# skokec/DAU-ConvNet

Measured on AMD Instinct MI355X. Metric: DAU fwd+bwd GSamples/s (N*H*W/s), higher is better.
Workload: dtype f32

## Files before the change

dau-convnet_amd/csrc/k_split_dot.hip:

```cpp
#include <algorithm>
#include <cfloat>

#include "dau_tiled.hpp"

namespace dau {

typedef _Float16 h8 __attribute__((ext_vector_type(8)));
typedef float f4s __attribute__((ext_vector_type(4)));

namespace {

constexpr int kSdWaves = 8;
constexpr int kSdAS = 2;
constexpr int kSdGT = 4;
constexpr int kSdSB = kSdWaves * kSdAS;
constexpr int kSdFB = 16;
constexpr int kSdR = 4;
constexpr int kSdRH = 4;
constexpr int kSdFlushItems = 16;
constexpr unsigned kVmcnt0 = 0x0F70, kVmcnt8 = 0x0F78;

inline size_t rup(size_t v, size_t a = 256) { return (v + a - 1) / a * a; }

struct SdGeom {
    int Hq, Wq, rq, cq, XTr, XTc, EYs, EXs, octs, nfb, nsb, ngb, items, chunks, per, NP;
};

SdGeom sd_geom(const SplitDotConfig& c) {
    const Shape& s = c.sh;
    SdGeom g{};
    g.Hq = (s.H + 1 + kSdRH - 1) / kSdRH * kSdRH;
    g.Wq = (s.W + 1 + c.RW - 1) / c.RW * c.RW;
    g.rq = g.Hq / kSdRH; g.cq = g.Wq / c.RW;
    g.XTr = g.Hq + 1; g.XTc = g.Wq + 1;
    g.EYs = g.Hq + 2 * kSdR; g.EXs = g.Wq + 2 * kSdR;
    g.octs = (s.N + 7) / 8;
    g.NP = (s.N + 1) / 2;
    g.nfb = (s.F + kSdFB - 1) / kSdFB;
    g.nsb = (s.S + kSdSB - 1) / kSdSB;
    g.ngb = (s.G + kSdGT - 1) / kSdGT;
    g.items = g.octs * g.rq * g.cq;
    const int per_chunk = g.nfb * g.nsb * g.ngb;
    int chunks = (1024 + per_chunk - 1) / per_chunk;
    chunks = std::max(1, std::min(chunks, g.items));
    g.per = (g.items + chunks - 1) / chunks;
    g.chunks = (g.items + g.per - 1) / g.per;
    return g;
}

struct SdLayout { size_t maxes_off, xk_off, xs_off, es_off, partial_off, total; };

SdLayout sd_layout(const SplitDotConfig& c, const SdGeom& g) {
    const Shape& s = c.sh;
    SdLayout l{};
    size_t off = 0;
    l.maxes_off = off; off += rup((size_t)(s.S * kNumK + s.F) * 4);
    l.xk_off = off; off += rup((size_t)g.NP * s.S * s.H * s.W * 32);
    l.xs_off = off; off += rup((size_t)g.octs * s.S * kNumK * g.XTr * g.XTc * 32 + 32);
    l.es_off = off; off += rup((size_t)g.octs * g.nfb * g.EYs * g.EXs * 256 * c.e_limbs);
    l.partial_off = off; off += rup((size_t)g.chunks * kNumK * s.S * s.G * s.F * 4);
    l.total = off;
    return l;
}

__device__ __forceinline__ int sd_shift(unsigned maxbits) {
    if (maxbits == 0u) return 0;
    const int e = (int)(maxbits >> 23) - 127;
    const int sh = 13 - e;
    return sh > 120 ? 120 : sh;
}

__device__ __forceinline__ bool finite_abs(float v, float* a) {
    *a = fabsf(v);
    return *a <= FLT_MAX;
}

#ifdef DAU_SD_STAGE_REF
__global__ void __launch_bounds__(256) sd_absmax_x_kernel(const float* __restrict__ xk, int NP, int S, int HW, int split,
                                                          unsigned* __restrict__ xmax, const Guard guard) {
    if (!guard_pass(guard)) return;
    const int s = blockIdx.x % S, part = blockIdx.x / S;
    float m[4] = {0.0f, 0.0f, 0.0f, 0.0f};
    const long per_np = (long)HW * 2;
    const long total = (long)NP * per_np;
    for (long i = part * 256L + threadIdx.x; i < total; i += 256L * split) {
        const long np = i / per_np, r = i - np * per_np;
        const float4 v = reinterpret_cast<const float4*>(xk + ((size_t)np * S + s) * HW * 8)[r];
        const int k0 = (int)(r & 1) * 2;
        float a;
        if (finite_abs(v.x, &a)) m[k0] = fmaxf(m[k0], a);
        if (finite_abs(v.y, &a)) m[k0] = fmaxf(m[k0], a);
        if (finite_abs(v.z, &a)) m[k0 + 1] = fmaxf(m[k0 + 1], a);
        if (finite_abs(v.w, &a)) m[k0 + 1] = fmaxf(m[k0 + 1], a);
    }
    __shared__ float red[4][256];
    for (int k = 0; k < 4; ++k) red[k][threadIdx.x] = m[k];
    __syncthreads();
    for (int w = 128; w >= 1; w >>= 1) {
        if ((int)threadIdx.x < w)
            for (int k = 0; k < 4; ++k) red[k][threadIdx.x] = fmaxf(red[k][threadIdx.x], red[k][threadIdx.x + w]);
        __syncthreads();
    }
    if (threadIdx.x < 4) atomicMax(&xmax[s * kNumK + threadIdx.x], __float_as_uint(red[threadIdx.x][0]));
}
#endif

__global__ void __launch_bounds__(256) sd_absmax_e_kernel(const float* __restrict__ dy, int N, int F, int HW, int split, int act,
                                                          unsigned* __restrict__ emax, const Guard guard) {
    if (!guard_pass(guard)) return;
    const int f = blockIdx.x % F, part = blockIdx.x / F;
    float m = 0.0f;
    const long total = (long)N * HW;
    for (long i = part * 256L + threadIdx.x; i < total; i += 256L * split) {
        const long n = i / HW, p = i - n * HW;
        float a;
        if (finite_abs(load_act(dy, ((long)n * F + f) * HW + p, act), &a)) m = fmaxf(m, a);
    }
    for (int o = 32; o >= 1; o >>= 1) m = fmaxf(m, __shfl_xor(m, o));
    if ((threadIdx.x & 63) == 0) atomicMax(&emax[f], __float_as_uint(m));
}

__global__ void __launch_bounds__(256) sd_absmax_nhwc_e_kernel(const float* __restrict__ dy, int N, int F, int HW, int split, int act,
                                                               unsigned* __restrict__ emax, const Guard guard) {
    if (!guard_pass(guard)) return;
    const int nfb = (F + 63) / 64;
    const int f = (blockIdx.x % nfb) * 64 + (threadIdx.x & 63), part = blockIdx.x / nfb;
    if (f >= F) return;
    float m = 0.0f;
    const long total = (long)N * HW;
    for (long i = part * 4L + (threadIdx.x >> 6); i < total; i += 4L * split) {
        float a;
        if (finite_abs(load_act(dy, i * F + f, act), &a)) m = fmaxf(m, a);
    }
    atomicMax(&emax[f], __float_as_uint(m));
}

__device__ __forceinline__ void split_limbs(float v, _Float16* hi, _Float16* lo) {
    const _Float16 h = (_Float16)v;
    const float hf = (float)h;
    *hi = h;
    *lo = (hf - hf == 0.0f) ? (_Float16)(v - hf) : (_Float16)0.0f;
}

__global__ void __launch_bounds__(256) sd_stage_x_kernel(const float* __restrict__ xk, const unsigned* __restrict__ xmax, int N,
                                                         int NP, int S, int H, int W, int octs, int XTr, int XTc,
                                                         h8* __restrict__ xs, const Guard guard) {
    if (!guard_pass(guard)) return;
    const long total = (long)octs * S * XTr * XTc;
    for (long idx = blockIdx.x * 256L + threadIdx.x; idx < total; idx += (long)gridDim.x * 256) {
        long t = idx;
        const int tx = (int)(t % XTc); t /= XTc;
        const int ty = (int)(t % XTr); t /= XTr;
        const int s = (int)(t % S);
        const int oct = (int)(t / S);
        const int y = ty - 1, x = tx - 1;
        const bool in = y >= 0 && y < H && x >= 0 && x < W;
        float v[4][8];
#pragma unroll
        for (int p = 0; p < 4; ++p) {
            const int np = oct * 4 + p;
            float4 a = make_float4(0.f, 0.f, 0.f, 0.f), b = a;
            if (in && np < NP) {
                const float4* src = reinterpret_cast<const float4*>(xk + ((((size_t)np * S + s) * H + y) * W + x) * 8);
                a = src[0]; b = src[1];
            }
            v[0][2 * p] = a.x; v[0][2 * p + 1] = a.y; v[1][2 * p] = a.z; v[1][2 * p + 1] = a.w;
            v[2][2 * p] = b.x; v[2][2 * p + 1] = b.y; v[3][2 * p] = b.z; v[3][2 * p + 1] = b.w;
        }
#pragma unroll
        for (int k = 0; k < 4; ++k) {
            const float sc = ldexpf(1.0f, sd_shift(xmax[s * kNumK + k]));
            h8 hi, lo;
#pragma unroll
            for (int i = 0; i < 8; ++i) {
                _Float16 h, l;
                split_limbs(v[k][i] * sc, &h, &l);
                hi[i] = h; lo[i] = l;
            }
            h8* dst = xs + ((((size_t)oct * S + s) * kNumK + k) * XTr * XTc + (size_t)ty * XTc + tx) * 2;
            dst[0] = hi; dst[1] = lo;
        }
    }
}

#ifndef DAU_SD_STAGE_REF
constexpr int kSeTX = 80;
__global__ void __launch_bounds__(256) sd_stage_e_kernel(const float* __restrict__ dy, const unsigned* __restrict__ emax, int N,
                                                         int F, int H, int W, int nfb, int EYs, int EXs, int nct, int TX,
                                                         int drop_col, int drop_row, int act, h8* __restrict__ es,
                                                         const Guard guard) {
    __shared__ h8 tile[kSeTX * 32];
    if (!guard_pass(guard)) return;
    int t = blockIdx.x;
    const int ct = t % nct; t /= nct;
    const int vy = t % EYs; t /= EYs;
    const int fb = t % nfb;
    const int oct = t / nfb;
    const int wlim = drop_col ? W - 1 : W, hlim = drop_row ? H - 1 : H;
    const int vx0 = ct * TX, nvx = min(TX, EXs - vx0);
    const int y = vy - (kSdR + 1);
    const int c0 = max(vx0, kSdR + 1), c1 = (y >= 0 && y < hlim) ? min(vx0 + nvx, kSdR + 1 + wlim) : c0;
    const int nd = max(c1 - c0, 0);
    for (int i = threadIdx.x; i < kSdFB * nd; i += 256) {
        const int fl = i / nd, vx = c0 + (i - fl * nd), x = vx - (kSdR + 1), lx = vx - vx0;
        const int f = fb * kSdFB + fl;
        const float sc = f < F ? ldexpf(1.0f, sd_shift(emax[f])) : 0.0f;
        float v[8];
#pragma unroll
        for (int n = 0; n < 8; ++n) {
            const int img = oct * 8 + n;
            v[n] = (f < F && img < N) ? load_act(dy, (((long)img * F + f) * H + y) * W + x, act) : 0.0f;
        }
        h8 hi, lo;
#pragma unroll
        for (int n = 0; n < 8; ++n) {
            _Float16 h, l;
            split_limbs(v[n] * sc, &h, &l);
            hi[n] = h; lo[n] = l;
        }
        tile[lx * 32 + (fl ^ (lx & 7))] = hi;
        tile[lx * 32 + ((kSdFB + fl) ^ (lx & 7))] = lo;
    }
    if (nd > 0) __syncthreads();
    h8* dst = es + ((((size_t)oct * nfb + fb) * EYs + vy) * EXs + vx0) * 32;
    for (int q = threadIdx.x; q < nvx * 32; q += 256) {
        const int lx = q >> 5, vx = vx0 + lx;
        h8 piece = {0, 0, 0, 0, 0, 0, 0, 0};
        if (vx >= c0 && vx < c1) piece = tile[lx * 32 + ((q & 31) ^ (lx & 7))];
        dst[q] = piece;
    }
}
#else
__global__ void __launch_bounds__(256) sd_stage_e_kernel(const float* __restrict__ dy, const unsigned* __restrict__ emax, int N,
                                                         int F, int H, int W, int octs, int nfb, int EYs, int EXs, int drop_col,
                                                         int drop_row, int act, int nhwc, h8* __restrict__ es, const Guard guard) {
    if (!guard_pass(guard)) return;
    const long total = (long)octs * nfb * EYs * EXs;
    const int wlim = drop_col ? W - 1 : W, hlim = drop_row ? H - 1 : H;
    for (long idx = blockIdx.x * 256L + threadIdx.x; idx < total; idx += (long)gridDim.x * 256) {
        long t = idx;
        const int vx = (int)(t % EXs); t /= EXs;
        const int vy = (int)(t % EYs); t /= EYs;
        const int fb = (int)(t % nfb);
        const int oct = (int)(t / nfb);
        const int y = vy - (kSdR + 1), x = vx - (kSdR + 1);
        const bool in = y >= 0 && y < hlim && x >= 0 && x < wlim;
        h8* dst = es + (size_t)idx * 32;
        for (int fl = 0; fl < kSdFB; ++fl) {
            const int f = fb * kSdFB + fl;
            const float sc = f < F ? ldexpf(1.0f, sd_shift(emax[f])) : 0.0f;
            h8 hi, lo;
#pragma unroll
            for (int i = 0; i < 8; ++i) {
                const int n = oct * 8 + i;
                const float v = (in && f < F && n < N) ? load_act(dy, nhwc ? nhwc_index(n, f, y, x, F, H, W) : (((long)n * F + f) * H + y) * W + x, act) : 0.0f;
                _Float16 h, l;
                split_limbs(v * sc, &h, &l);
                hi[i] = h; lo[i] = l;
            }
            dst[fl] = hi; dst[kSdFB + fl] = lo;
        }
    }
}
#endif

constexpr int kSe1TX = 80;
__global__ void __launch_bounds__(256) sd_stage_e1_kernel(const float* __restrict__ dy, const unsigned* __restrict__ emax, int N,
                                                          int F, int H, int W, int nfb, int EYs, int EXs, int nct, int TX,
                                                          int drop_col, int drop_row, int act, h8* __restrict__ es,
                                                          const Guard guard) {
    __shared__ h8 tile[kSe1TX * kSdFB];
    if (!guard_pass(guard)) return;
    int t = blockIdx.x;
    const int ct = t % nct; t /= nct;
    const int vy = t % EYs; t /= EYs;
    const int fb = t % nfb;
    const int oct = t / nfb;
    const int wlim = drop_col ? W - 1 : W, hlim = drop_row ? H - 1 : H;
    const int vx0 = ct * TX, nvx = min(TX, EXs - vx0);
    const int y = vy - (kSdR + 1);
    const int c0 = max(vx0, kSdR + 1), c1 = (y >= 0 && y < hlim) ? min(vx0 + nvx, kSdR + 1 + wlim) : c0;
    const int nd = max(c1 - c0, 0);
    for (int i = threadIdx.x; i < kSdFB * nd; i += 256) {
        const int fl = i / nd, vx = c0 + (i - fl * nd), x = vx - (kSdR + 1), lx = vx - vx0;
        const int f = fb * kSdFB + fl;
        const float sc = f < F ? ldexpf(1.0f, sd_shift(emax[f])) : 0.0f;
        float v[8];
#pragma unroll
        for (int n = 0; n < 8; ++n) {
            const int img = oct * 8 + n;
            v[n] = (f < F && img < N) ? load_act(dy, (((long)img * F + f) * H + y) * W + x, act) : 0.0f;
        }
        h8 hi;
#pragma unroll
        for (int n = 0; n < 8; ++n) hi[n] = (_Float16)(v[n] * sc);
        tile[lx * kSdFB + (fl ^ (lx & 7))] = hi;
    }
    if (nd > 0) __syncthreads();
    h8* dst = es + ((((size_t)oct * nfb + fb) * EYs + vy) * EXs + vx0) * kSdFB;
    for (int q = threadIdx.x; q < nvx * kSdFB; q += 256) {
        const int lx = q >> 4, vx = vx0 + lx;
        h8 piece = {0, 0, 0, 0, 0, 0, 0, 0};
        if (vx >= c0 && vx < c1) piece = tile[lx * kSdFB + ((q & 15) ^ (lx & 7))];
        dst[q] = piece;
    }
}

template <int LIMBS>
__global__ void __launch_bounds__(256) sd_stage_nhwc_e_kernel(const float* __restrict__ dy, const unsigned* __restrict__ emax, int N,
                                                              int F, int H, int W, int nfb, int EYs, int EXs, int nct, int TX,
                                                              int drop_col, int drop_row, int act, h8* __restrict__ es,
                                                              const Guard guard) {
    if (!guard_pass(guard)) return;
    int t = blockIdx.x;
    const int ct = t % nct; t /= nct;
    const int vy = t % EYs; t /= EYs;
    const int fb = t % nfb;
    const int oct = t / nfb;
    const int wlim = drop_col ? W - 1 : W, hlim = drop_row ? H - 1 : H;
    const int vx0 = ct * TX, nvx = min(TX, EXs - vx0);
    const int y = vy - (kSdR + 1);
    const int c0 = max(vx0, kSdR + 1), c1 = (y >= 0 && y < hlim) ? min(vx0 + nvx, kSdR + 1 + wlim) : c0;
    h8* dst = es + ((((size_t)oct * nfb + fb) * EYs + vy) * EXs + vx0) * (kSdFB * LIMBS);
    for (int i = threadIdx.x; i < nvx * kSdFB; i += 256) {
        const int lx = i / kSdFB, fl = i - lx * kSdFB, vx = vx0 + lx, x = vx - (kSdR + 1);
        const int f = fb * kSdFB + fl;
        const bool in = vx >= c0 && vx < c1 && f < F;
        const float sc = f < F ? ldexpf(1.0f, sd_shift(emax[f])) : 0.0f;
        float v[8];
#pragma unroll
        for (int n = 0; n < 8; ++n) {
            const int img = oct * 8 + n;
            const bool ok = in && img < N;
            v[n] = mask_act(load_act(dy, ok ? nhwc_index(img, f, y, x, F, H, W) : 0, act), ok);
        }
        h8 hi, lo;
#pragma unroll
        for (int n = 0; n < 8; ++n) {
            if constexpr (LIMBS == 2) {
                _Float16 h, l;
                split_limbs(v[n] * sc, &h, &l);
                hi[n] = h; lo[n] = l;
            } else {
                hi[n] = (_Float16)(v[n] * sc);
            }
        }
        dst[lx * (kSdFB * LIMBS) + fl] = hi;
        if constexpr (LIMBS == 2) dst[lx * (kSdFB * LIMBS) + kSdFB + fl] = lo;
    }
}

struct SdArgs {
    const h8* xs;
    const char* es;
    const unsigned* xmax;
    const unsigned* emax;
    const UnitRef* table;
    float* partial;
    int S, F, G;
    int nfb, nsb, ngb, per, items, rq, cq, XTr, XTc, EYs, EXs;
    Guard guard;
};

__device__ __forceinline__ void sd_glds16(const char* src, unsigned dst) {
    unsigned keep;
    asm volatile("s_mov_b32 %0, m0\n\ts_mov_b32 m0, %2\n\ts_nop 0\n\tglobal_load_lds_dwordx4 %1, off\n\ts_mov_b32 m0, %0"
                 : "=&s"(keep) : "v"(src), "s"(dst) : "memory");
}

#ifndef DAU_SD_STEP_LOADS
__device__ __forceinline__ h8 sd_next_col(h8 cur, h8 nxt, int dx) {
    typedef int i4s __attribute__((ext_vector_type(4)));
    const i4s c = __builtin_bit_cast(i4s, cur), n = __builtin_bit_cast(i4s, nxt);
    i4s r;
#pragma unroll
    for (int d = 0; d < 4; ++d)
        r[d] = __builtin_amdgcn_update_dpp(0, dx ? c[d] : n[d], 0xB1 , 0xF, 0xF, true);
    return __builtin_bit_cast(h8, r);
}
#endif

template <int RW, int EL>
__device__ __forceinline__ void sd_dot_body(const SdArgs& a) {
    extern __shared__ __attribute__((aligned(16))) char lds[];
    if (!guard_pass(a.guard)) return;
    constexpr int WL = RW + 2 * kSdR, WR = kSdRH + 2 * kSdR;
    constexpr int kRing = WR + kSdRH;
    constexpr int PB = EL * 256;
    constexpr unsigned RB = WL * PB;
    constexpr int kRowPieces = (RB + 1023) / 1024;
    static_assert((kRing & (kRing - 1)) == 0, "ring slot = (origin + row) & (kRing - 1)");
    static_assert(RW % 2 == 0, "A fragment sets by the parity of the K step / of the pair of K steps");
#ifdef DAU_SD_STEP_LOADS
    constexpr int kSdAStride = 2;
#else
    constexpr int kSdAStride = 4;
#endif
    static_assert((size_t)kRing * RB <= 160 * 1024, "the ring fills the LDS");
    int t = blockIdx.x;
    const int gb = t % a.ngb; t /= a.ngb;
    const int sb = t % a.nsb; t /= a.nsb;
    const int fb = t % a.nfb; t /= a.nfb;
    const int chunk = t;
    const int it0 = chunk * a.per, it1 = min(it0 + a.per, a.items);
    const int lane = threadIdx.x & 63, wave = threadIdx.x >> 6;
    const int wave_u = __builtin_amdgcn_readfirstlane(wave);
    const int fl = lane & 15, j = lane >> 4;
    const int f = fb * kSdFB + fl;
    const bool f_ok = f < a.F;
    const unsigned lds0 = (unsigned)(uintptr_t)(__attribute__((address_space(3))) char*)lds;
    const int m = lane & 15, ak = m >> 2, ady = (m >> 1) & 1, adx = m & 1;
    const size_t xplane = (size_t)a.XTr * a.XTc;
    unsigned aoff[kSdAS];
    int sidx[kSdAS];
    bool s_ok[kSdAS];
    unsigned uw[kSdAS][kSdGT];
    f4s wb[kSdAS][kSdGT];
    float run[kSdAS][kSdGT];
#pragma unroll
    for (int i = 0; i < kSdAS; ++i) {
        const int s = sb * kSdSB + wave * kSdAS + i;
        s_ok[i] = s < a.S;
        sidx[i] = s_ok[i] ? s : a.S - 1;
        aoff[i] = (unsigned)((((size_t)sidx[i] * kNumK + ak) * xplane + (size_t)(j + ady) * a.XTc + adx) * 2);
#pragma unroll
        for (int gg = 0; gg < kSdGT; ++gg) {
            const int g = gb * kSdGT + gg;
            UnitRef u{0, 0, 0.0f, 0.0f, 0.0f, 0.0f};
            if (s_ok[i] && g < a.G && f_ok) u = a.table[((size_t)sidx[i] * a.G + g) * a.F + f];
            uw[i][gg] = (unsigned)(j - u.oy + kSdR) | (unsigned)((kSdR - u.ox) * PB + fl * 16) << 4;
            wb[i][gg] = f4s{u.w00, u.w01, u.w10, u.w11};
            run[i][gg] = 0.0f;
        }
    }
    int shx[kSdAS];
    const int she = f_ok ? sd_shift(a.emax[f]) : 0;
#pragma unroll
    for (int i = 0; i < kSdAS; ++i) shx[i] = sd_shift(a.xmax[sidx[i] * kNumK + j]);
    auto flush = [&]() {
#pragma unroll
        for (int i = 0; i < kSdAS; ++i) {
#pragma unroll
            for (int gg = 0; gg < kSdGT; ++gg) {
                const int g = gb * kSdGT + gg;
                if (s_ok[i] && g < a.G && f_ok) {
                    const float v = ldexpf(ldexpf(run[i][gg], -shx[i]), -she);
                    float* dst = a.partial + ((((size_t)chunk * kNumK + j) * a.S + sidx[i]) * a.G + g) * a.F + f;
                    __hip_atomic_fetch_add(dst, v, __ATOMIC_RELAXED, __HIP_MEMORY_SCOPE_AGENT);
                }
                run[i][gg] = 0.0f;
            }
        }
    };
    const int per_oct = a.rq * a.cq;
    auto item_off = [&](int item) {
        const int oct = item / per_oct, reg = item - oct * per_oct, rx = reg / a.rq, ry = reg - rx * a.rq;
        return ((size_t)oct * a.S * kNumK * xplane + (size_t)(ry * kSdRH) * a.XTc + (size_t)rx * RW) * 2;
    };
    auto fill = [&](int oct, int ry, int rx, int w0, int nrows, int origin) {
#ifndef DAU_SD_DIAG_NOFILL
        const char* src = a.es + ((((size_t)oct * a.nfb + fb) * a.EYs + (size_t)(ry * kSdRH + w0)) * a.EXs + (size_t)rx * RW) * PB;
        for (int u = wave_u; u < nrows * kRowPieces; u += kSdWaves) {
            const int rr = u / kRowPieces, pc = u - rr * kRowPieces;
            const unsigned within = pc * 1024 + lane * 16;
            const unsigned slot = (unsigned)(origin + w0 + rr) & (kRing - 1);
            if (within < RB) sd_glds16(src + (size_t)rr * a.EXs * PB + within, lds0 + slot * RB + pc * 1024);
        }
#endif
    };
    h8 ahi[2][kSdAS], alo[2][kSdAS];
    if (it0 < it1) {
#pragma unroll
        for (int p = 0; p < 2; ++p)
#pragma unroll
            for (int i = 0; i < kSdAS; ++i) {
                const h8* ap = a.xs + item_off(it0) + (size_t)p * kSdAStride + aoff[i];
                ahi[p][i] = ap[0]; alo[p][i] = ap[1];
            }
    }
    int since_flush = 0;
    int origin = 0;
    for (int it = it0; it < it1; ++it) {
        const int oct = it / per_oct, reg = it - oct * per_oct, rx = reg / a.rq, ry = reg - rx * a.rq;
        __builtin_amdgcn_s_waitcnt(kVmcnt8);
        __syncthreads();
        if (it > it0 && ry > 0) {
            origin = (origin + kSdRH) & (kRing - 1);
        } else {
            origin = 0;
            fill(oct, ry, rx, 0, WR, 0);
            __builtin_amdgcn_s_waitcnt(kVmcnt0);
            __syncthreads();
        }
        if (it + 1 < it1 && ry + 1 < a.rq) fill(oct, ry, rx, WR, kSdRH, origin);
        int base[kSdAS][kSdGT];
#pragma unroll
        for (int i = 0; i < kSdAS; ++i)
#pragma unroll
            for (int gg = 0; gg < kSdGT; ++gg)
                base[i][gg] = (int)((((unsigned)origin + (uw[i][gg] & 15u)) & (kRing - 1)) * RB + (uw[i][gg] >> 4));
#ifdef DAU_SD_DIAG_AFIXED
        const size_t ioff = item_off(it0), ioff_next = ioff;
#else
        const size_t ioff = item_off(it);
        const size_t ioff_next = item_off(it + 1 < it1 ? it + 1 : it);
#endif
        f4s part[kSdAS][kSdGT];
#pragma unroll
        for (int i = 0; i < kSdAS; ++i)
#pragma unroll
            for (int gg = 0; gg < kSdGT; ++gg) part[i][gg] = f4s{0.0f, 0.0f, 0.0f, 0.0f};
#ifdef DAU_SD_DIAG_NOA
#define SD_LOAD_A(P, i, an)
#else
#define SD_LOAD_A(P, i, an) { const h8* ap = a.xs + (an) + aoff[i]; ahi[P][i] = ap[0]; alo[P][i] = ap[1]; }
#endif
#define SD_READ_B(i, bh, bl)                                                                                    \
    _Pragma("unroll") for (int gg = 0; gg < kSdGT; ++gg) {                                                      \
        const char* bp = lds + base[i][gg] + k * PB;                                                            \
        bh[gg] = *reinterpret_cast<const h8*>(bp);                                                              \
        if constexpr (EL == 2) bl[gg] = *reinterpret_cast<const h8*>(bp + 256);                                 \
    }
#define SD_GROUP(i, AH, AL, bh, bl, AFTER)                                                                      \
    __builtin_amdgcn_sched_barrier(0);                                                                          \
    _Pragma("unroll") for (int gg = 0; gg < kSdGT; ++gg) {                                                      \
        part[i][gg] = __builtin_amdgcn_mfma_f32_16x16x32_f16(AH, bh[gg], part[i][gg], 0, 0, 0);                 \
        part[i][gg] = __builtin_amdgcn_mfma_f32_16x16x32_f16(AL, bh[gg], part[i][gg], 0, 0, 0);                 \
        if constexpr (EL == 2) part[i][gg] = __builtin_amdgcn_mfma_f32_16x16x32_f16(AH, bl[gg], part[i][gg], 0, 0, 0); \
    }                                                                                                           \
    AFTER                                                                                                       \
    __builtin_amdgcn_sched_barrier(0);
#define SD_STEP(kk, AH, AL, AFTER0, AFTER1)                                                                     \
    {                                                                                                           \
        const int k = (kk);                                                                                     \
        h8 b0h[kSdGT], b0l[kSdGT], b1h[kSdGT], b1l[kSdGT];                                                      \
        SD_READ_B(0, b0h, b0l)                                                                                  \
        SD_READ_B(1, b1h, b1l)                                                                                  \
        SD_GROUP(0, AH[0], AL[0], b0h, b0l, AFTER0)                                                             \
        SD_GROUP(1, AH[1], AL[1], b1h, b1l, AFTER1)                                                             \
    }
        static_assert(kSdAS == 2, "two groups per K step");
#ifdef DAU_SD_STEP_LOADS
#define SD_STEP1(P, kk)                                                                                         \
    {                                                                                                           \
        const size_t an = (kk) + 2 < RW ? ioff + (size_t)((kk) + 2) * 2 : ioff_next + (size_t)((kk) + 2 - RW) * 2; \
        (void)an;                                                                                               \
        SD_STEP(kk, ahi[P], alo[P], SD_LOAD_A(P, 0, an), SD_LOAD_A(P, 1, an))                                   \
    }
#pragma unroll 1
        for (int k2 = 0; k2 < RW; k2 += 2) {
            SD_STEP1(0, k2)
            SD_STEP1(1, k2 + 1)
        }
#undef SD_STEP1
#else
        h8 aqh[kSdAS], aql[kSdAS];
#define SD_NEXT_COL(P, i)                                                                                       \
    aqh[i] = sd_next_col(ahi[P][i], ahi[1 - (P)][i], adx);                                                      \
    aql[i] = sd_next_col(alo[P][i], alo[1 - (P)][i], adx);
#define SD_PAIR(P, rr)                                                                                          \
    {                                                                                                           \
        const size_t an = ioff + (size_t)((rr) + 2) * 4;                                                        \
        (void)an;                                                                                               \
        SD_STEP(2 * (rr), ahi[P], alo[P], SD_NEXT_COL(P, 0) SD_LOAD_A(P, 0, an), SD_NEXT_COL(P, 1) SD_LOAD_A(P, 1, an)) \
        SD_STEP(2 * (rr) + 1, aqh, aql, , )                                                                     \
    }
#define SD_PAIR_LAST(P, rr)                                                                                     \
    {                                                                                                           \
        SD_STEP(2 * (rr), ahi[P], alo[P], SD_NEXT_COL(P, 0) SD_LOAD_A(0, 0, ioff_next), SD_NEXT_COL(P, 1) SD_LOAD_A(0, 1, ioff_next)) \
        SD_STEP(2 * (rr) + 1, aqh, aql, SD_LOAD_A(1, 0, ioff_next + 4), SD_LOAD_A(1, 1, ioff_next + 4))         \
    }
        constexpr int kPairs = RW / 2, kLoopPairs = (kPairs - 1) / 2 * 2;
#pragma unroll 1
        for (int r2 = 0; r2 < kLoopPairs; r2 += 2) {
            SD_PAIR(0, r2)
            SD_PAIR(1, r2 + 1)
        }
        if constexpr (kPairs - kLoopPairs == 2) {
            SD_PAIR(0, kPairs - 2)
            SD_PAIR_LAST(1, kPairs - 1)
        } else {
            SD_PAIR_LAST(0, kPairs - 1)
        }
#undef SD_NEXT_COL
#undef SD_PAIR
#undef SD_PAIR_LAST
#endif
#undef SD_READ_B
#undef SD_GROUP
#undef SD_LOAD_A
#undef SD_STEP
#pragma unroll
        for (int i = 0; i < kSdAS; ++i)
#pragma unroll
            for (int gg = 0; gg < kSdGT; ++gg) {
                const int g = gb * kSdGT + gg;
                const bool ok = s_ok[i] && g < a.G && f_ok;
                const f4s p = part[i][gg], w = wb[i][gg];
                float v = w[0] * p[0];
                v = fmaf(w[1], p[1], v);
                v = fmaf(w[2], p[2], v);
                v = fmaf(w[3], p[3], v);
                run[i][gg] += ok ? v : 0.0f;
            }
        if (++since_flush == kSdFlushItems) { flush(); since_flush = 0; }
    }
    asm volatile("s_waitcnt vmcnt(0)" ::: "memory");
    if (since_flush) flush();
}

template <int RW>
__global__ void __launch_bounds__(kSdWaves * 64) __attribute__((amdgpu_waves_per_eu(2, 2))) split_gather_dot_kernel(const SdArgs a) {
    sd_dot_body<RW, 2>(a);
}

template <int RW>
__global__ void __launch_bounds__(kSdWaves * 64) __attribute__((amdgpu_waves_per_eu(2, 2))) sd_e1_dot_kernel(const SdArgs a) {
    sd_dot_body<RW, 1>(a);
}

template <int RW, int EL>
void launch_sd(hipStream_t st, const SdArgs* a, int grid) {
    auto kern = [] { if constexpr (EL == 2) return split_gather_dot_kernel<RW>; else return sd_e1_dot_kernel<RW>; }();
    const size_t lds = (size_t)(2 * kSdRH + 2 * kSdR) * (RW + 2 * kSdR) * 256 * EL;
    if (!a) { (void)hipFuncSetAttribute(reinterpret_cast<const void*>(kern), hipFuncAttributeMaxDynamicSharedMemorySize, 160 * 1024); return; }
    hipLaunchKernelGGL(kern, dim3(grid), dim3(kSdWaves * 64), lds, st, *a);
}
void dispatch_sd(int RW, int e_limbs, hipStream_t st, const SdArgs* a, int grid) {
    if (e_limbs == 1) {
        if (RW == 10) launch_sd<10, 1>(st, a, grid);
        else launch_sd<12, 1>(st, a, grid);
    } else {
        if (RW == 10) launch_sd<10, 2>(st, a, grid);
        else launch_sd<12, 2>(st, a, grid);
    }
}

}

bool split_dot_configure(const Shape& sh, int blur_k, int act, SplitDotConfig* cfg) {
    int best = 0;
    long best_cost = 1L << 40;
    for (int rw = 12; rw >= 10; rw -= 2) {
        const long wq = (sh.W + 1 + rw - 1) / rw * rw;
        const long cost = wq * (rw + 2) * (60 / rw);
        if (cost < best_cost) { best_cost = cost; best = rw; }
    }
    if ((size_t)(2 * kSdRH + 2 * kSdR) * (best + 2 * kSdR) * 512 > 160 * 1024) return false;
    if (!blur4_pack_fits(blur_k, sh.H, sh.W)) return false;
    SplitDotConfig c{};
    c.sh = sh; c.blur_k = blur_k; c.RW = best; c.act = act;
#ifdef DAU_SD_BF16_E2
    c.e_limbs = 2;
#else
    c.e_limbs = act == kActBF16 ? 1 : 2;
#endif
    const SdGeom g = sd_geom(c);
    if ((long)g.EXs * 512 * 32 > (1L << 31)) return false;
    *cfg = c;
    return true;
}

size_t split_dot_workspace_bytes(const SplitDotConfig& c) { return sd_layout(c, sd_geom(c)).total; }

void split_dot_init(const SplitDotConfig& c) {
    dispatch_sd(c.RW, c.e_limbs, nullptr, nullptr, 0);
#ifndef DAU_SD_STAGE_REF
    blur4_pack_init(c.blur_k, true, c.nhwc != 0);
#else
    blur4_pack_init(c.blur_k, false, c.nhwc != 0);
#endif
}

void split_dot_prepare(hipStream_t st, const SplitDotConfig& c, const float* x, const float* dy, const float* filters,
                       int drop_col, int drop_row, void* workspace, const Guard& guard) {
    const SdGeom g = sd_geom(c);
    const SdLayout l = sd_layout(c, g);
    const Shape& s = c.sh;
    char* ws = static_cast<char*>(workspace);
    unsigned* xmax = reinterpret_cast<unsigned*>(ws + l.maxes_off);
    unsigned* emax = xmax + s.S * kNumK;
    float* xk = reinterpret_cast<float*>(ws + l.xk_off);
    (void)hipMemsetAsync(xmax, 0, (size_t)(s.S * kNumK + s.F) * 4, st);
    (void)hipMemsetAsync(ws + l.partial_off, 0, (size_t)g.chunks * kNumK * s.S * s.G * s.F * 4, st);
    const int HW = s.H * s.W;
#ifndef DAU_SD_STAGE_REF
    launch_blur4_pack(st, x, filters, s.N, s.S, s.S, s.H, s.W, s.H, s.W, c.blur_k, c.act, xk, guard, xmax, c.nhwc != 0);
#else
    launch_blur4_pack(st, x, filters, s.N, s.S, s.S, s.H, s.W, s.H, s.W, c.blur_k, c.act, xk, guard, nullptr, c.nhwc != 0);
    const int xsplit = std::max(1, std::min(16, 2048 / std::max(1, s.S)));
    hipLaunchKernelGGL(sd_absmax_x_kernel, dim3(s.S * xsplit), dim3(256), 0, st, xk, g.NP, s.S, HW, xsplit, xmax, guard);
#endif
    if (c.nhwc) {
        const int nfb64 = (s.F + 63) / 64;
        const int esplit = (int)std::max(1L, std::min((long)(2048 / nfb64), ((long)s.N * HW + 3) / 4));
        hipLaunchKernelGGL(sd_absmax_nhwc_e_kernel, dim3(nfb64 * esplit), dim3(256), 0, st, dy, s.N, s.F, HW, esplit, c.act, emax, guard);
    } else {
        const int esplit = std::max(1, std::min(16, 2048 / std::max(1, s.F)));
        hipLaunchKernelGGL(sd_absmax_e_kernel, dim3(s.F * esplit), dim3(256), 0, st, dy, s.N, s.F, HW, esplit, c.act, emax, guard);
    }
    hipLaunchKernelGGL(sd_stage_x_kernel, dim3(8192), dim3(256), 0, st, xk, xmax, s.N, g.NP, s.S, s.H, s.W, g.octs, g.XTr, g.XTc,
                       reinterpret_cast<h8*>(ws + l.xs_off), guard);
    if (c.e_limbs == 1) {
        const int nct = (g.EXs + kSe1TX - 1) / kSe1TX, tx = (g.EXs + nct - 1) / nct;
        if (c.nhwc) {
            hipLaunchKernelGGL(sd_stage_nhwc_e_kernel<1>, dim3((unsigned)(g.octs * g.nfb * g.EYs * nct)), dim3(256), 0, st, dy, emax, s.N, s.F,
                               s.H, s.W, g.nfb, g.EYs, g.EXs, nct, tx, drop_col, drop_row, c.act, reinterpret_cast<h8*>(ws + l.es_off), guard);
            return;
        }
        hipLaunchKernelGGL(sd_stage_e1_kernel, dim3((unsigned)(g.octs * g.nfb * g.EYs * nct)), dim3(256), 0, st, dy, emax, s.N, s.F,
                           s.H, s.W, g.nfb, g.EYs, g.EXs, nct, tx, drop_col, drop_row, c.act, reinterpret_cast<h8*>(ws + l.es_off), guard);
        return;
    }
#ifndef DAU_SD_STAGE_REF
    const int nct = (g.EXs + kSeTX - 1) / kSeTX, tx = (g.EXs + nct - 1) / nct;
    if (c.nhwc) {
        hipLaunchKernelGGL(sd_stage_nhwc_e_kernel<2>, dim3((unsigned)(g.octs * g.nfb * g.EYs * nct)), dim3(256), 0, st, dy, emax, s.N, s.F,
                           s.H, s.W, g.nfb, g.EYs, g.EXs, nct, tx, drop_col, drop_row, c.act, reinterpret_cast<h8*>(ws + l.es_off), guard);
        return;
    }
    hipLaunchKernelGGL(sd_stage_e_kernel, dim3((unsigned)(g.octs * g.nfb * g.EYs * nct)), dim3(256), 0, st, dy, emax, s.N, s.F, s.H,
                       s.W, g.nfb, g.EYs, g.EXs, nct, tx, drop_col, drop_row, c.act, reinterpret_cast<h8*>(ws + l.es_off), guard);
#else
    hipLaunchKernelGGL(sd_stage_e_kernel, dim3(4096), dim3(256), 0, st, dy, emax, s.N, s.F, s.H, s.W, g.octs, g.nfb, g.EYs, g.EXs,
                       drop_col, drop_row, c.act, c.nhwc, reinterpret_cast<h8*>(ws + l.es_off), guard);
#endif
}

void split_dot_run(hipStream_t st, const SplitDotConfig& c, const UnitRef* table, float* r4, void* workspace, const Guard& guard) {
    const SdGeom g = sd_geom(c);
    const SdLayout l = sd_layout(c, g);
    const Shape& s = c.sh;
    char* ws = static_cast<char*>(workspace);
    SdArgs a{};
    a.xs = reinterpret_cast<const h8*>(ws + l.xs_off);
    a.es = ws + l.es_off;
    a.xmax = reinterpret_cast<const unsigned*>(ws + l.maxes_off);
    a.emax = a.xmax + s.S * kNumK;
    a.table = table;
    a.partial = reinterpret_cast<float*>(ws + l.partial_off);
    a.S = s.S; a.F = s.F; a.G = s.G;
    a.nfb = g.nfb; a.nsb = g.nsb; a.ngb = g.ngb; a.per = g.per; a.items = g.items; a.rq = g.rq; a.cq = g.cq;
    a.XTr = g.XTr; a.XTc = g.XTc; a.EYs = g.EYs; a.EXs = g.EXs;
    a.guard = guard;
    dispatch_sd(c.RW, c.e_limbs, st, &a, g.chunks * g.nfb * g.nsb * g.ngb);
    launch_dot_reduce(st, a.partial, 1, (long)kNumK * s.S * s.G * s.F, s.G, s.F, s.G, g.chunks, g.chunks, s.G, false, r4, guard);
}

}
```

Measured before the change: 0.01815.

## Fuse separable blur and limb staging into two-pass row-walking kernels

Adds a row-walking kernel that computes the separable blurred input planes on the fly with packed FMA. It runs twice: once to find per-channel absolute maxima, and once to split the values into scaled fp16 limbs and store them straight into the staged layout. This skips the intermediate xk buffer and its write/read round trip through memory. The cost is recomputing the blur in both passes and using small 64-thread blocks with wave-level LDS sync, and it applies only to NCHW with blur sizes 5, 7 or 9.

New measurement: 0.01861 (median of 6 runs). 2.5% higher.

```diff
diff --git a/dau-convnet_amd/csrc/k_split_dot.hip b/dau-convnet_amd/csrc/k_split_dot.hip
--- a/dau-convnet_amd/csrc/k_split_dot.hip
+++ b/dau-convnet_amd/csrc/k_split_dot.hip
@@ -181,6 +181,181 @@
             dst[0] = hi; dst[1] = lo;
         }
     }
+}
+
+constexpr int kXwCols = 16;
+constexpr int kXwAhead = 3;
+constexpr int kXwOut = kNumK * kXwCols * 2 * 4;
+struct XkWalkArgs {
+    const float* x;
+    const float* taps;
+    unsigned* xmax;
+    h8* xs;
+    int N, S, H, W, XTr, XTc, nct, act;
+    Guard guard;
+};
+
+__device__ __forceinline__ void xw_wave_sync() {
+    __builtin_amdgcn_fence(__ATOMIC_RELEASE, "wavefront");
+    __builtin_amdgcn_wave_barrier();
+    __builtin_amdgcn_fence(__ATOMIC_ACQUIRE, "wavefront");
+}
+
+typedef float f2 __attribute__((ext_vector_type(2)));
+template <int N, class F>
+__device__ __forceinline__ void xw_unroll(F&& f) {
+    [&]<int... I>(std::integer_sequence<int, I...>) { (f(std::integral_constant<int, I>{}), ...); }(std::make_integer_sequence<int, N>{});
+}
+template <int HALF>
+__device__ __forceinline__ f2 xw_fma_tap(f2 a, unsigned long taps, f2 c) {
+    f2 d;
+    if constexpr (HALF == 0) asm("v_pk_fma_f32 %0, %1, %2, %3 op_sel_hi:[1,0,1]" : "=v"(d) : "v"(a), "s"(taps), "v"(c));
+    else asm("v_pk_fma_f32 %0, %1, %2, %3 op_sel:[0,1,0] op_sel_hi:[1,1,1]" : "=v"(d) : "v"(a), "s"(taps), "v"(c));
+    return d;
+}
+
+template <int K, bool STORE, int AF>
+__device__ __forceinline__ void sd_xk_walk(const XkWalkArgs& a, float* lds) {
+    typedef int i4s __attribute__((ext_vector_type(4)));
+    typedef _Float16 h2s __attribute__((ext_vector_type(2)));
+    typedef typename RawAct<AF>::type Raw;
+    constexpr int KR = (K - 1) / 2, CW = kXwCols + 2 * KR, NL = (8 * CW + 63) / 64, kBuf = NL * 64;
+    static_assert(kXwAhead < K, "the rows in flight are slots of the unrolled loop");
+    int t = blockIdx.x;
+    const int ct = t % a.nct; t /= a.nct;
+    const int s = t % a.S, oct = t / a.S;
+    const int lane = threadIdx.x, c = lane >> 2, p = lane & 3;
+    const int H = a.H, W = a.W;
+    const int tx0 = ct * kXwCols, x = tx0 + c - 1;
+    const float* tp[6] = {a.taps + kTapGX * kTapPitch, a.taps + kTapAX * kTapPitch, a.taps + kTapCX * kTapPitch,
+                          a.taps + kTapGY * kTapPitch, a.taps + kTapAY * kTapPitch, a.taps + kTapBY * kTapPitch};
+    unsigned long tq[6][(K + 1) / 2];
+#pragma unroll
+    for (int f = 0; f < 6; ++f)
+#pragma unroll
+        for (int j = 0; j < (K + 1) / 2; ++j) tq[f][j] = __builtin_bit_cast(unsigned long, f2{tp[f][2 * j], tp[f][2 * j + 1]});
+    long poff[NL];
+    int lw[NL];
+    float mf[NL];
+    bool keep[NL];
+#pragma unroll
+    for (int l = 0; l < NL; ++l) {
+        const int tt = l * 64 + lane, tc = tt < 8 * CW ? tt : 8 * CW - 1;
+        const int img = tc / CW, col = tc - img * CW;
+        const int n = oct * 8 + img;
+        const bool second = (n & 1) && n - 1 < a.N;
+        const int src = n < a.N ? n : second ? n - 1 : oct * 8;
+        const int xx = tx0 - 1 - KR + col;
+        keep[l] = tt < 8 * CW && xx >= 0 && xx < W && (n < a.N || second);
+        mf[l] = n < a.N ? 1.0f : 0.0f;
+        poff[l] = ((long)src * a.S + s) * H * W + (xx < 0 ? 0 : xx < W ? xx : W - 1);
+        lw[l] = tt < 8 * CW ? col * 8 + img : tt;
+    }
+    constexpr unsigned kKeyZero = 1u << 24;
+    unsigned km[4] = {kKeyZero, kKeyZero, kKeyZero, kKeyZero}, seen[4] = {0u, 0u, 0u, 0u};
+    float sc[4] = {1.0f, 1.0f, 1.0f, 1.0f};
+#pragma unroll
+    for (int k = 0; k < 4; ++k) {
+        if constexpr (STORE) sc[k] = ldexpf(1.0f, sd_shift(a.xmax[s * kNumK + k]));
+        else seen[k] = __hip_atomic_load(a.xmax + s * kNumK + k, __ATOMIC_RELAXED, __HIP_MEMORY_SCOPE_AGENT);
+    }
+    const int steps = (a.XTr + K - 1 + K - 1) / K * K;
+    Raw rv[K][NL];
+    f2 hr[K][3];
+#pragma unroll
+    for (int i = 0; i < K; ++i)
+#pragma unroll
+        for (int f = 0; f < 3; ++f) hr[i][f] = f2{0.0f, 0.0f};
+    auto load_row = [&](int u, Raw* dst) {
+        const int r = u - 1 - KR, rc = r < 0 ? 0 : r < H ? r : H - 1;
+#pragma unroll
+        for (int l = 0; l < NL; ++l) dst[l] = load_raw<AF>(a.x, poff[l] + (long)rc * W);
+    };
+#pragma unroll
+    for (int d = 0; d < kXwAhead; ++d) load_row(d, rv[d]);
+    const size_t plane = (size_t)a.XTr * a.XTc;
+    h8* const out = a.xs + ((size_t)(oct * a.S + s) * kNumK + (lane >> 5)) * plane * 2 + (size_t)tx0 * 2 + (lane & 31);
+    const bool col_in = tx0 + ((lane & 31) >> 1) < a.XTc;
+    float* obuf = lds + 2 * kBuf;
+    auto step = [&](auto pc, int u) {
+        constexpr int P = decltype(pc)::value;
+        load_row(u + kXwAhead, rv[(P + kXwAhead) % K]);
+        const int r = u - 1 - KR;
+        const bool row_in = r >= 0 && r < H;
+        float* buf = lds + (u & 1) * kBuf;
+#pragma unroll
+        for (int l = 0; l < NL; ++l) buf[lw[l]] = mask_act(mf[l] * act_of(rv[P][l]), keep[l] && row_in);
+        xw_wave_sync();
+        f2 h[3] = {{0.0f, 0.0f}, {0.0f, 0.0f}, {0.0f, 0.0f}};
+        xw_unroll<K>([&](auto ic) {
+            constexpr int I = decltype(ic)::value, i = I;
+            const f2 v = *reinterpret_cast<const f2*>(buf + (c + i) * 8 + 2 * p);
+#pragma unroll
+            for (int f = 0; f < 3; ++f) h[f] = xw_fma_tap<I & 1>(v, tq[f][I / 2], h[f]);
+        });
+#pragma unroll
+        for (int f = 0; f < 3; ++f) hr[P][f] = h[f];
+        const int ty = u - (K - 1), y = ty - 1;
+        f2 o[4] = {{0.0f, 0.0f}, {0.0f, 0.0f}, {0.0f, 0.0f}, {0.0f, 0.0f}};
+        xw_unroll<K>([&](auto jc) {
+            constexpr int J = decltype(jc)::value, sl = (P + 1 + J) % K;
+            const unsigned long gy = tq[3][J / 2], ay = tq[4][J / 2], by = tq[5][J / 2];
+            const f2 b1 = hr[sl][0], b2 = hr[sl][1], b3 = hr[sl][2];
+            o[0] = xw_fma_tap<J & 1>(b1, gy, o[0]);
+            o[1] = xw_fma_tap<J & 1>(b2, gy, o[1]);
+            o[2] = xw_fma_tap<J & 1>(b1, ay, o[2]);
+            o[3] = xw_fma_tap<J & 1>(b3, gy, o[3]);
+            o[3] = xw_fma_tap<J & 1>(b1, by, o[3]);
+        });
+        const bool in = y >= 0 && y < H && x >= 0 && x < W;
+#pragma unroll
+        for (int k = 0; k < 4; ++k) {
+            const float v0 = mask_act(o[k].x, in), v1 = mask_act(o[k].y, in);
+            if constexpr (!STORE) {
+                km[k] = max(max(km[k], (__float_as_uint(v0) << 1) + kKeyZero), (__float_as_uint(v1) << 1) + kKeyZero);
+            } else {
+                h2s hi, lo;
+                _Float16 hh, ll;
+                split_limbs(v0 * sc[k], &hh, &ll);
+                hi[0] = hh; lo[0] = ll;
+                split_limbs(v1 * sc[k], &hh, &ll);
+                hi[1] = hh; lo[1] = ll;
+                obuf[(k * kXwCols + c) * 8 + p] = __builtin_bit_cast(float, hi);
+                obuf[(k * kXwCols + c) * 8 + 4 + p] = __builtin_bit_cast(float, lo);
+            }
+        }
+        if constexpr (STORE) {
+            xw_wave_sync();
+            const i4s piece0 = *reinterpret_cast<const i4s*>(obuf + lane * 4);
+            const i4s piece1 = *reinterpret_cast<const i4s*>(obuf + (64 + lane) * 4);
+            if (col_in && ty >= 0 && ty < a.XTr) {
+                h8* dst = out + (size_t)ty * a.XTc * 2;
+                dst[0] = __builtin_bit_cast(h8, piece0);
+                dst[2 * plane * 2] = __builtin_bit_cast(h8, piece1);
+            }
+        }
+    };
+#pragma unroll 1
+    for (int u0 = 0; u0 < steps; u0 += K) {
+        xw_unroll<K>([&](auto pc) { step(pc, u0 + decltype(pc)::value); });
+    }
+    if constexpr (!STORE) {
+#pragma unroll
+        for (int k = 0; k < 4; ++k) {
+            unsigned m = km[k];
+            for (int w = 32; w >= 1; w >>= 1) m = max(m, (unsigned)__shfl_xor((int)m, w));
+            const unsigned bits = (m - kKeyZero) >> 1;
+            if (lane == 0 && bits > seen[k]) atomicMax(a.xmax + s * kNumK + k, bits);
+        }
+    }
+}
+
+template <int K, bool STORE>
+__global__ void __launch_bounds__(64) sd_xk_walk_kernel(const XkWalkArgs a) {
+    constexpr int kBuf = (8 * (kXwCols + K - 1) + 63) / 64 * 64;
+    __shared__ __attribute__((aligned(16))) float lds[2 * kBuf + (STORE ? kXwOut : 0)];
+    if (!guard_pass(a.guard)) return;
+    with_act(a.act, [&](auto actc) { sd_xk_walk<K, STORE, decltype(actc)::value>(a, lds); });
 }
 
 #ifndef DAU_SD_STAGE_REF
@@ -626,6 +801,33 @@
     if (!a) { (void)hipFuncSetAttribute(reinterpret_cast<const void*>(kern), hipFuncAttributeMaxDynamicSharedMemorySize, 160 * 1024); return; }
     hipLaunchKernelGGL(kern, dim3(grid), dim3(kSdWaves * 64), lds, st, *a);
 }
+bool sd_walks(const SplitDotConfig& c) {
+#if defined(DAU_SD_XK_COPY) || defined(DAU_SD_STAGE_REF)
+    return false;
+#else
+    const SdGeom g = sd_geom(c);
+    const long nct = (g.XTc + kXwCols - 1) / kXwCols;
+    return !c.nhwc && (c.blur_k == 5 || c.blur_k == 7 || c.blur_k == 9) && (long)g.octs * c.sh.S * nct < (1L << 31);
+#endif
+}
+template <int K, bool STORE>
+void launch_xk_walk(hipStream_t st, const XkWalkArgs& a, int grid) {
+    hipLaunchKernelGGL((sd_xk_walk_kernel<K, STORE>), dim3(grid), dim3(64), 0, st, a);
+}
+template <bool STORE>
+void dispatch_xk_walk(hipStream_t st, const SplitDotConfig& c, const SdGeom& g, const float* x, const float* filters, unsigned* xmax,
+                      h8* xs, const Guard& guard) {
+    XkWalkArgs a{};
+    a.x = x; a.taps = filters + kTaps1dOffset; a.xmax = xmax; a.xs = xs;
+    a.N = c.sh.N; a.S = c.sh.S; a.H = c.sh.H; a.W = c.sh.W; a.XTr = g.XTr; a.XTc = g.XTc; a.act = c.act;
+    a.nct = (g.XTc + kXwCols - 1) / kXwCols;
+    a.guard = guard;
+    const int grid = g.octs * c.sh.S * a.nct;
+    if (c.blur_k == 5) launch_xk_walk<5, STORE>(st, a, grid);
+    else if (c.blur_k == 7) launch_xk_walk<7, STORE>(st, a, grid);
+    else launch_xk_walk<9, STORE>(st, a, grid);
+}
+
 void dispatch_sd(int RW, int e_limbs, hipStream_t st, const SdArgs* a, int grid) {
     if (e_limbs == 1) {
         if (RW == 10) launch_sd<10, 1>(st, a, grid);
@@ -684,8 +886,11 @@
     (void)hipMemsetAsync(xmax, 0, (size_t)(s.S * kNumK + s.F) * 4, st);
     (void)hipMemsetAsync(ws + l.partial_off, 0, (size_t)g.chunks * kNumK * s.S * s.G * s.F * 4, st);
     const int HW = s.H * s.W;
+    const bool walks = sd_walks(c);
+    h8* xs = reinterpret_cast<h8*>(ws + l.xs_off);
 #ifndef DAU_SD_STAGE_REF
-    launch_blur4_pack(st, x, filters, s.N, s.S, s.S, s.H, s.W, s.H, s.W, c.blur_k, c.act, xk, guard, xmax, c.nhwc != 0);
+    if (walks) dispatch_xk_walk<false>(st, c, g, x, filters, xmax, xs, guard);
+    else launch_blur4_pack(st, x, filters, s.N, s.S, s.S, s.H, s.W, s.H, s.W, c.blur_k, c.act, xk, guard, xmax, c.nhwc != 0);
 #else
     launch_blur4_pack(st, x, filters, s.N, s.S, s.S, s.H, s.W, s.H, s.W, c.blur_k, c.act, xk, guard, nullptr, c.nhwc != 0);
     const int xsplit = std::max(1, std::min(16, 2048 / std::max(1, s.S)));
@@ -699,8 +904,8 @@
         const int esplit = std::max(1, std::min(16, 2048 / std::max(1, s.F)));
         hipLaunchKernelGGL(sd_absmax_e_kernel, dim3(s.F * esplit), dim3(256), 0, st, dy, s.N, s.F, HW, esplit, c.act, emax, guard);
     }
-    hipLaunchKernelGGL(sd_stage_x_kernel, dim3(8192), dim3(256), 0, st, xk, xmax, s.N, g.NP, s.S, s.H, s.W, g.octs, g.XTr, g.XTc,
-                       reinterpret_cast<h8*>(ws + l.xs_off), guard);
+    if (walks) dispatch_xk_walk<true>(st, c, g, x, filters, xmax, xs, guard);
+    else hipLaunchKernelGGL(sd_stage_x_kernel, dim3(8192), dim3(256), 0, st, xk, xmax, s.N, g.NP, s.S, s.H, s.W, g.octs, g.XTr, g.XTc, xs, guard);
     if (c.e_limbs == 1) {
         const int nct = (g.EXs + kSe1TX - 1) / kSe1TX, tx = (g.EXs + nct - 1) / nct;
         if (c.nhwc) {
```
